# allenai/satlas-super-resolution

Measured on AMD Instinct MI355X. Metric: G+D train-step images/sec, higher is better.
Workload: dtype fp32h

## Files before the change

satlas_super_resolution_amd/csrc/conv_thin.hip:

```cpp
#include "common.h"
#include <cstdlib>

namespace {

constexpr int CT_TH = 8, CT_TW = 32, CT_PH = CT_TH + 2, CT_PW = CT_TW + 2, CT_NPIX = CT_PH * CT_PW;
typedef __bf16 bf16x2t __attribute__((ext_vector_type(2)));

__device__ __forceinline__ float ct_dot8(const u32x4& a, const u32x4& b, float acc) {
    const unsigned a0 = a.x, a1 = a.y, a2 = a.z, a3 = a.w, b0 = b.x, b1 = b.y, b2 = b.z, b3 = b.w;
    acc = __builtin_amdgcn_fdot2_f32_bf16(__builtin_bit_cast(bf16x2t, a0), __builtin_bit_cast(bf16x2t, b0), acc, false);
    acc = __builtin_amdgcn_fdot2_f32_bf16(__builtin_bit_cast(bf16x2t, a1), __builtin_bit_cast(bf16x2t, b1), acc, false);
    acc = __builtin_amdgcn_fdot2_f32_bf16(__builtin_bit_cast(bf16x2t, a2), __builtin_bit_cast(bf16x2t, b2), acc, false);
    acc = __builtin_amdgcn_fdot2_f32_bf16(__builtin_bit_cast(bf16x2t, a3), __builtin_bit_cast(bf16x2t, b3), acc, false);
    return acc;
}

template <int NCO>
__global__ __launch_bounds__(256) void conv_thin_kernel(const ssr_conv_desc d) {
    extern __shared__ __attribute__((aligned(16))) char smem[];
    const int tid = threadIdx.x;
    const int cin = d.Cin, nvec = cin >> 3;
    const int rowb = cin * 2 + 16;
    const int tiles_x = (d.Gw + CT_TW - 1) / CT_TW, tiles_y = (d.Gh + CT_TH - 1) / CT_TH;
    int b = blockIdx.x;
    const int tx_i = b % tiles_x; b /= tiles_x;
    const int ty_i = b % tiles_y;
    const int n = b / tiles_y;
    const int gy0 = ty_i * CT_TH, gx0 = tx_i * CT_TW;
    const __bf16* __restrict__ xg = reinterpret_cast<const __bf16*>(d.x.p);
    const __bf16* __restrict__ wg = reinterpret_cast<const __bf16*>(d.w);
    {
        constexpr int NSV = (CT_NPIX * 8 + 255) / 256;
        const int total = CT_NPIX * nvec;
        const float rn = 1.0f / (float)nvec;
        u32x4 sv[NSV];
        unsigned okm = 0;
#pragma unroll
        for (int q = 0; q < NSV; ++q) {
            const int v = tid + q * 256;
            const int pix = (int)(((float)v + 0.5f) * rn), part = v - pix * nvec;
            const int py = pix / CT_PW, px = pix - py * CT_PW;
            const int ly = gy0 + py - 1, lx = gx0 + px - 1;
            const bool ok = v < total && ly >= 0 && ly < d.Hi && lx >= 0 && lx < d.Wi;
            okm |= ok ? 1u << q : 0u;
            sv[q] = *reinterpret_cast<const u32x4*>(xg + (ok ? ((size_t)(n * d.Hi + ly) * d.Wi + lx) * d.x.cs + d.x.coff + part * 8 : (size_t)0));
        }
#pragma unroll
        for (int q = 0; q < NSV; ++q) {
            const int v = tid + q * 256;
            const int pix = (int)(((float)v + 0.5f) * rn), part = v - pix * nvec;
            if (v < total) *reinterpret_cast<u32x4*>(smem + pix * rowb + part * 16) = (okm >> q) & 1u ? sv[q] : u32x4{0u, 0u, 0u, 0u};
        }
    }
    __syncthreads();
    const int ty = tid >> 5, tx = tid & 31;
    float acc[NCO];
#pragma unroll
    for (int c = 0; c < NCO; ++c) acc[c] = 0.f;
    const char* pb = smem + (ty * CT_PW + tx) * rowb;
    for (int tap = 0; tap < 9; ++tap) {
        const char* pr = pb + ((tap / 3) * CT_PW + tap % 3) * rowb;
        for (int k = 0; k < nvec; ++k) {
            const u32x4 xv = *reinterpret_cast<const u32x4*>(pr + k * 16);
            const __bf16* wk = wg + ((size_t)((k >> 2) * 9 + tap) * d.CoutPad) * 32 + (k & 3) * 8;
#pragma unroll
            for (int c = 0; c < NCO; ++c) {
                const u32x4 wv = *reinterpret_cast<const u32x4*>(wk + c * 32);
                acc[c] = ct_dot8(xv, wv, acc[c]);
            }
        }
    }
    const int gy = gy0 + ty, gx = gx0 + tx;
    if (gy >= d.Gh || gx >= d.Gw) return;
    const size_t pp = (size_t)(n * d.Ho + gy * d.oys + d.oyo) * d.Wo + gx * d.oxs + d.oxo;
    __bf16* __restrict__ yp = reinterpret_cast<__bf16*>(d.y.p);
    __bf16* __restrict__ y0p = reinterpret_cast<__bf16*>(d.y0.p);
    __bf16* __restrict__ y1p = reinterpret_cast<__bf16*>(d.y1.p);
    const __bf16* __restrict__ r1p = reinterpret_cast<const __bf16*>(d.r1.p);
    const __bf16* __restrict__ r2p = reinterpret_cast<const __bf16*>(d.r2.p);
    const __bf16* __restrict__ mp = reinterpret_cast<const __bf16*>(d.m.p);
#pragma unroll
    for (int c = 0; c < NCO; ++c) {
        if (c >= d.Cout) break;
        float v = acc[c] + (d.bias ? d.bias[c] : 0.f);
        if (d.act == SSR_ACT_LRELU) v = lrelu(v);
        v *= d.alpha;
        if (y0p) y0p[pp * d.y0.cs + d.y0.coff + c] = (__bf16)v;
        if (r1p && c < d.r1_nc) v += d.beta1 * (float)r1p[pp * d.r1.cs + d.r1.coff + c];
        if (r2p && c < d.r2_nc) v += d.beta2 * (float)r2p[pp * d.r2.cs + d.r2.coff + c];
        if (d.accumulate) v += (float)yp[pp * d.y.cs + d.y.coff + c];
        if (y1p) y1p[pp * d.y1.cs + d.y1.coff + c] = (__bf16)v;
        if (mp && c >= d.m_c0 && c < d.m_c1) v *= lrelu_grad_from_out((float)mp[pp * d.m.cs + d.m.coff + c]);
        yp[pp * d.y.cs + d.y.coff + c] = (__bf16)v;
    }
}

constexpr int CTF_CB = 32, CTF_ROWB = CTF_CB * 4 + 16;
constexpr int CTF_PATCH = CT_NPIX * CTF_ROWB;

template <int NCO, int X3>
__global__ __launch_bounds__(256) void conv_thin_f32_kernel(const ssr_conv_desc d) {
    constexpr int NCOP = NCO == 1 ? 1 : NCO <= 4 ? 4 : 8;
    extern __shared__ __attribute__((aligned(16))) char smem[];
    float* wl = reinterpret_cast<float*>(smem + CTF_PATCH);
    const int tid = threadIdx.x;
    const int cin = d.Cin, cin16 = (cin + 15) & ~15;
    const int tiles_x = (d.Gw + CT_TW - 1) / CT_TW, tiles_y = (d.Gh + CT_TH - 1) / CT_TH;
    int b = blockIdx.x;
    const int tx_i = b % tiles_x; b /= tiles_x;
    const int ty_i = b % tiles_y;
    const int n = b / tiles_y;
    const int gy0 = ty_i * CT_TH, gx0 = tx_i * CT_TW;
    const float* __restrict__ xg = reinterpret_cast<const float*>(d.x.p);
    const char* __restrict__ wg = reinterpret_cast<const char*>(d.w);
    const int ty = tid >> 5, tx = tid & 31;
    const char* pb = smem + (ty * CT_PW + tx) * CTF_ROWB;
    float acc[NCOP];
#pragma unroll
    for (int c = 0; c < NCOP; ++c) acc[c] = 0.f;
    constexpr int NSV = (CT_NPIX * 8 + 255) / 256;
    int sofs[NSV];
#pragma unroll
    for (int q = 0; q < NSV; ++q) {
        const int v = tid + q * 256, pix = v >> 3;
        const int py = pix / CT_PW, px = pix - py * CT_PW;
        const int ly = gy0 + py - 1, lx = gx0 + px - 1;
        const bool ok = v < CT_NPIX * 8 && ly >= 0 && ly < d.Hi && lx >= 0 && lx < d.Wi;
        sofs[q] = ok ? ((n * d.Hi + ly) * d.Wi + lx) * d.x.cs + d.x.coff + (v & 7) * 4 : -1;
    }
    u32x4 sv[NSV];
    auto load_pass = [&](int c0) {
#pragma unroll
        for (int q = 0; q < NSV; ++q) {
            const bool ok = sofs[q] >= 0 && c0 + ((tid + q * 256) & 7) * 4 < cin;
            sv[q] = *reinterpret_cast<const u32x4*>(xg + (ok ? sofs[q] + c0 : 0));
        }
    };
    auto store_pass = [&](int c0) {
#pragma unroll
        for (int q = 0; q < NSV; ++q) {
            const int v = tid + q * 256;
            const bool ok = sofs[q] >= 0 && c0 + (v & 7) * 4 < cin;
            if (v < CT_NPIX * 8) *reinterpret_cast<u32x4*>(smem + (v >> 3) * CTF_ROWB + (v & 7) * 16) = ok ? sv[q] : u32x4{0u, 0u, 0u, 0u};
        }
    };
    load_pass(0);
    for (int e = tid; e < 9 * cin16 * NCOP; e += 256) {
        const int c = e % NCOP, q = e / NCOP, ci = q % cin16, tap = q / cin16;
        float w = 0.f;
        if (c < NCO) {
            const char* row = wg + ((size_t)((ci >> 4) * 9 + tap) * d.CoutPad + c) * 64;
            if (X3 == 2) {
                const _Float16 h = reinterpret_cast<const _Float16*>(row)[ci & 15], l = reinterpret_cast<const _Float16*>(row)[16 + (ci & 15)];
                w = ((float)h + (float)l) * SSR_F32H_UNSCALE;
            } else if (X3 == 1) {
                const unsigned short h = reinterpret_cast<const unsigned short*>(row)[ci & 15], l = reinterpret_cast<const unsigned short*>(row)[16 + (ci & 15)];
                w = __builtin_bit_cast(float, (unsigned)h << 16) + __builtin_bit_cast(float, (unsigned)l << 16);
            } else {
                w = reinterpret_cast<const float*>(row)[ci & 15];
            }
        }
        wl[e] = w;
    }
    store_pass(0);
    __syncthreads();
    for (int c0 = 0; c0 < cin; c0 += CTF_CB) {
        const bool more = c0 + CTF_CB < cin;
        if (more) load_pass(c0 + CTF_CB);
        const int nk = (min(cin16 - c0, CTF_CB)) >> 2;
        for (int tap = 0; tap < 9; ++tap) {
            const char* pr = pb + ((tap / 3) * CT_PW + tap % 3) * CTF_ROWB;
            const float* wt = wl + (tap * cin16 + c0) * NCOP;
            for (int k = 0; k < nk; ++k) {
                const f32x4 xv = *reinterpret_cast<const f32x4*>(pr + k * 16);
                if constexpr (NCOP == 1) {
                    const f32x4 w = *reinterpret_cast<const f32x4*>(wt + 4 * k);
                    acc[0] = fmaf(xv.x, w.x, acc[0]); acc[0] = fmaf(xv.y, w.y, acc[0]);
                    acc[0] = fmaf(xv.z, w.z, acc[0]); acc[0] = fmaf(xv.w, w.w, acc[0]);
                } else {
#pragma unroll
                    for (int j = 0; j < 4; ++j) {
                        const float xj = j == 0 ? xv.x : j == 1 ? xv.y : j == 2 ? xv.z : xv.w;
#pragma unroll
                        for (int c4 = 0; c4 < NCOP / 4; ++c4) {
                            const f32x4 w = *reinterpret_cast<const f32x4*>(wt + (4 * k + j) * NCOP + 4 * c4);
                            acc[4 * c4] = fmaf(xj, w.x, acc[4 * c4]); acc[4 * c4 + 1] = fmaf(xj, w.y, acc[4 * c4 + 1]);
                            acc[4 * c4 + 2] = fmaf(xj, w.z, acc[4 * c4 + 2]); acc[4 * c4 + 3] = fmaf(xj, w.w, acc[4 * c4 + 3]);
                        }
                    }
                }
            }
        }
        if (more) {
            __syncthreads();
            store_pass(c0 + CTF_CB);
            __syncthreads();
        }
    }
    const int gy = gy0 + ty, gx = gx0 + tx;
    if (gy >= d.Gh || gx >= d.Gw) return;
    const size_t pp = (size_t)(n * d.Ho + gy * d.oys + d.oyo) * d.Wo + gx * d.oxs + d.oxo;
    float* __restrict__ yp = reinterpret_cast<float*>(d.y.p);
    float* __restrict__ y0p = reinterpret_cast<float*>(d.y0.p);
    float* __restrict__ y1p = reinterpret_cast<float*>(d.y1.p);
    const float* __restrict__ r1p = reinterpret_cast<const float*>(d.r1.p);
    const float* __restrict__ r2p = reinterpret_cast<const float*>(d.r2.p);
    const float* __restrict__ mp = reinterpret_cast<const float*>(d.m.p);
#pragma unroll
    for (int c = 0; c < NCO; ++c) {
        if (c >= d.Cout) break;
        float v = acc[c] + (d.bias ? d.bias[c] : 0.f);
        if (d.act == SSR_ACT_LRELU) v = lrelu(v);
        else if (d.act == SSR_ACT_RELU) v = fmaxf(v, 0.f);
        v *= d.alpha;
        if (y0p) y0p[pp * d.y0.cs + d.y0.coff + c] = v;
        if (r1p && c < d.r1_nc) v += d.beta1 * r1p[pp * d.r1.cs + d.r1.coff + c];
        if (r2p && c < d.r2_nc) v += d.beta2 * r2p[pp * d.r2.cs + d.r2.coff + c];
        if (d.accumulate) v += yp[pp * d.y.cs + d.y.coff + c];
        if (y1p) y1p[pp * d.y1.cs + d.y1.coff + c] = v;
        if (mp && c >= d.m_c0 && c < d.m_c1) {
            const float mv = mp[pp * d.m.cs + d.m.coff + c];
            v *= d.m_relu ? (mv > 0.f ? 1.f : 0.f) : lrelu_grad_from_out(mv);
        }
        yp[pp * d.y.cs + d.y.coff + c] = v;
    }
}

template <int NCO, int X3>
int launch_thin_f32(const ssr_conv_desc& d, hipStream_t st) {
    constexpr int NCOP = NCO == 1 ? 1 : NCO <= 4 ? 4 : 8;
    const size_t lds = (size_t)CTF_PATCH + (size_t)9 * ((d.Cin + 15) & ~15) * NCOP * 4;
    auto kern = conv_thin_f32_kernel<NCO, X3>;
    static bool attr_done[SSR_MAX_DEVICES] = {};
    const int attr_dev = ssr_device_ordinal();
    if (!attr_done[attr_dev]) {
        hipError_t e = hipFuncSetAttribute(reinterpret_cast<const void*>(kern), hipFuncAttributeMaxDynamicSharedMemorySize, CTF_PATCH + 9 * 64 * 8 * 4);
        if (e != hipSuccess) return (int)e;
        attr_done[attr_dev] = true;
    }
    const int tiles = d.N * ((d.Gh + CT_TH - 1) / CT_TH) * ((d.Gw + CT_TW - 1) / CT_TW);
    hipLaunchKernelGGL(kern, dim3(tiles), dim3(256), lds, st, d);
    SSR_LAUNCH_CHECK();
    return SSR_OK;
}
template <int X3>
int launch_thin_f32_by_cout(const ssr_conv_desc& d, hipStream_t st) {
    if (d.Cout == 1) return launch_thin_f32<1, X3>(d, st);
    if (d.Cout <= 3) return launch_thin_f32<3, X3>(d, st);
    if (d.Cout == 4) return launch_thin_f32<4, X3>(d, st);
    return launch_thin_f32<8, X3>(d, st);
}

template <int NCO>
int launch_thin(const ssr_conv_desc& d, hipStream_t st) {
    const size_t lds = (size_t)CT_NPIX * (d.Cin * 2 + 16);
// ... 50 lines not shown
```

satlas_super_resolution_amd/csrc/misc.hip:

```cpp
#include "common.h"
#include "adam.h"
#include <cstdlib>

namespace {

__device__ __forceinline__ float wave_sum(float v) {
#pragma unroll
    for (int o = 32; o > 0; o >>= 1) v += __shfl_down(v, o, 64);
    return v;
}
__device__ __forceinline__ float block_sum(float v, float* sh) {
    const int lane = threadIdx.x & 63, w = threadIdx.x >> 6, nw = (blockDim.x + 63) >> 6;
    v = wave_sum(v);
    __syncthreads();
    if (lane == 0) sh[w] = v;
    __syncthreads();
    float s = 0.f;
    if (threadIdx.x < 64) {
        s = (threadIdx.x < nw) ? sh[threadIdx.x] : 0.f;
        s = wave_sum(s);
        if (threadIdx.x == 0) sh[0] = s;
    }
    __syncthreads();
    return sh[0];
}

template <typename T, int X3>
__device__ __forceinline__ void put_packed(T* __restrict__ dst, size_t idx, int ck, float v) {
    if (X3 == 2 && ck == 16) {
        _Float16* row = reinterpret_cast<_Float16*>(dst) + (idx >> 4) * 32;
        const float vs = v * SSR_F32H_WSCALE;
        const _Float16 h = (_Float16)vs;
        row[idx & 15] = h;
        row[16 + (idx & 15)] = (_Float16)(vs - (float)h);
    } else if (X3 == 1 && ck == 16) {
        __bf16* row = reinterpret_cast<__bf16*>(dst) + (idx >> 4) * 32;
        const __bf16 h = (__bf16)v;
        row[idx & 15] = h;
        row[16 + (idx & 15)] = (__bf16)(v - (float)h);
    } else {
        dst[idx] = from_f32<T>(v);
    }
}

template <typename T, int X3 = 0>
__global__ __launch_bounds__(256) void pack_kernel(const ssr_pack_item* __restrict__ items) {
    const ssr_pack_item it = items[blockIdx.y];
    const int KK = it.KH * it.KW;
    const float inv = it.inv_scale ? 1.0f / it.inv_scale[0] : 1.0f;
    const int stride = gridDim.x * blockDim.x;
    const int t0 = blockIdx.x * blockDim.x + threadIdx.x;
    if (it.dst_fwd) {
        T* __restrict__ dst = reinterpret_cast<T*>(it.dst_fwd);
        const int ck = it.ck_fwd, total = it.CoutPad * it.CinPad;
        for (int t = t0; t < total; t += stride) {
            const int cc = t % ck, q = t / ck;
            const int co = q % it.CoutPad, chunk = q / it.CoutPad;
            const int ci = chunk * ck + cc;
            const bool ok = co < it.Cout && ci < it.Cin;
            const float* __restrict__ sp = it.src + ((size_t)co * it.Cin + ci) * KK;
            if (it.fwd_s2d) {
                const int nch = it.CinPad / ck;
                for (int tap = 0; tap < 16; ++tap) {
                    const int ky = tap >> 2, kx = tap & 3, q = (ky & 1) * 2 + (kx & 1), tt = (ky >> 1) * 2 + (kx >> 1);
                    put_packed<T, X3>(dst, ((((size_t)q * nch + chunk) * 4 + tt) * it.CoutPad + co) * ck + cc, ck, ok ? sp[tap] * inv : 0.f);
                }
                continue;
            }
            const size_t dp = ((size_t)chunk * KK * it.CoutPad + co) * ck + cc;
            for (int tap = 0; tap < KK; ++tap) put_packed<T, X3>(dst, dp + (size_t)tap * it.CoutPad * ck, ck, ok ? sp[tap] * inv : 0.f);
        }
    }
    if (it.dst_dgrad) {
        T* __restrict__ dst = reinterpret_cast<T*>(it.dst_dgrad);
        const int ck = it.ck_dgrad, total = it.CinPadO * it.CoutPadI;
        for (int t = t0; t < total; t += stride) {
            const int cc = t % ck, q = t / ck;
            const int o = q % it.CinPadO, chunk = q / it.CinPadO;
            const int k = chunk * ck + cc;
            const bool ok = k < it.Cout && o < it.Cin;
            const float* __restrict__ sp = it.src + ((size_t)k * it.Cin + o) * KK;
            if (it.stride == 1) {
                const size_t dp = ((size_t)chunk * KK * it.CinPadO + o) * ck + cc;
                for (int tap = 0; tap < KK; ++tap)
                    put_packed<T, X3>(dst, dp + (size_t)tap * it.CinPadO * ck, ck, ok ? sp[KK - 1 - tap] * inv : 0.f);
            } else {
                const size_t per_cls = (size_t)4 * it.CinPadO * it.CoutPadI;
                for (int cls = 0; cls < 4; ++cls)
                    for (int tt = 0; tt < 4; ++tt) {
                        const int py = cls >> 1, px = cls & 1, ty = tt >> 1, tx = tt & 1;
                        const int ky = py ? 2 - 2 * ty : 3 - 2 * ty, kx = px ? 2 - 2 * tx : 3 - 2 * tx;
                        put_packed<T, X3>(dst, cls * per_cls + (((size_t)chunk * 4 + tt) * it.CinPadO + o) * ck + cc, ck,
                                          ok ? sp[ky * 4 + kx] * inv : 0.f);
                    }
            }
        }
    }
}

template <typename T, int X3 = 0>
__global__ __launch_bounds__(256) void pack_seg_kernel(const ssr_pack_seg* __restrict__ items) {
    const ssr_pack_seg it = items[blockIdx.y];
    T* __restrict__ dst = reinterpret_cast<T*>(it.dst);
    const int total = it.Cout * it.rows_pad;
    for (int t = blockIdx.x * blockDim.x + threadIdx.x; t < total; t += gridDim.x * blockDim.x) {
        const int kk = t % it.Cout, o = t / it.Cout;
        const int k = it.kbase + kk, chunk = k / it.ck, cc = k - chunk * it.ck;
        const bool ok = o < it.nci;
        const float* __restrict__ sp = it.src + ((size_t)kk * it.Cin + it.ci0 + o) * 9;
        const size_t dp = ((size_t)chunk * 9 * it.rows_pad + o) * it.ck + cc;
#pragma unroll
        for (int tap = 0; tap < 9; ++tap) put_packed<T, X3>(dst, dp + (size_t)tap * it.rows_pad * it.ck, it.ck, ok ? it.scale * sp[8 - tap] : 0.f);
    }
}

template <typename T>
__global__ __launch_bounds__(256) void add_views_kernel(ssr_view dst, ssr_view src, long npix, int C) {
    T* __restrict__ d = reinterpret_cast<T*>(dst.p);
    const T* __restrict__ s = reinterpret_cast<const T*>(src.p);
    const long total = npix * C;
    for (long e = (long)blockIdx.x * blockDim.x + threadIdx.x; e < total; e += (long)gridDim.x * blockDim.x) {
        const long p = e / C;
        const int c = (int)(e - p * C);
        const long di = p * dst.cs + dst.coff + c;
        d[di] = from_f32<T>(to_f32(d[di]) + to_f32(s[p * src.cs + src.coff + c]));
    }
}

template <typename T>
__global__ __launch_bounds__(256) void nchw_to_nhwc_kernel(const float* __restrict__ src, int N, int C, int H, int W,
                                                           ssr_view dst, int s, int up, float scale) {
    const int C2 = C * s * s, H2 = H / s * up, W2 = W / s * up;
    const long total = (long)N * H2 * W2 * C2;
    T* __restrict__ d = reinterpret_cast<T*>(dst.p);
    for (long e = (long)blockIdx.x * blockDim.x + threadIdx.x; e < total; e += (long)gridDim.x * blockDim.x) {
        const int c2 = (int)(e % C2);
        long q = e / C2;
        const int x = (int)(q % W2); q /= W2;
        const int y = (int)(q % H2);
        const int n = (int)(q / H2);
        const int ys = y / up, xs = x / up;
        const int c = c2 / (s * s), i = (c2 / s) % s, j = c2 % s;
        const float v = src[(((long)n * C + c) * H + ys * s + i) * W + xs * s + j] * scale;
        d[(((long)n * H2 + y) * W2 + x) * dst.cs + dst.coff + c2] = from_f32<T>(v);
    }
}

template <typename T>
__global__ __launch_bounds__(256) void nhwc_to_nchw_kernel(ssr_view src, float* __restrict__ dst, int N, int C, int H,
                                                           int W) {
    const long total = (long)N * C * H * W;
    const T* __restrict__ s = reinterpret_cast<const T*>(src.p);
    for (long e = (long)blockIdx.x * blockDim.x + threadIdx.x; e < total; e += (long)gridDim.x * blockDim.x) {
        const int x = (int)(e % W);
        long q = e / W;
        const int y = (int)(q % H); q /= H;
        const int c = (int)(q % C);
        const int n = (int)(q / C);
        dst[e] = to_f32(s[(((long)n * H + y) * W + x) * src.cs + src.coff + c]);
    }
}

template <typename T>
__global__ __launch_bounds__(256) void fill_kernel(T* __restrict__ p, long n, float v) {
    for (long e = (long)blockIdx.x * blockDim.x + threadIdx.x; e < n; e += (long)gridDim.x * blockDim.x)
        p[e] = from_f32<T>(v);
}

__device__ __forceinline__ void bil_src(int o, int n_in, int& i0, int& i1, float& l0, float& l1) {
    float s = 0.5f * (float)o - 0.25f;
    s = s < 0.f ? 0.f : s;
    i0 = (int)s;
    i1 = i0 + (i0 < n_in - 1 ? 1 : 0);
    l1 = s - (float)i0;
    l0 = 1.f - l1;
}

template <typename T> struct VecIO;
template <> struct VecIO<float> {
    static constexpr int N = 4;
    static __device__ __forceinline__ void load(const float* p, float (&f)[4]) {
        const f32x4 v = *reinterpret_cast<const f32x4*>(p);
#pragma unroll
        for (int k = 0; k < 4; ++k) f[k] = v[k];
    }
    static __device__ __forceinline__ void store(float* p, const float (&f)[4]) {
        f32x4 v;
#pragma unroll
        for (int k = 0; k < 4; ++k) v[k] = f[k];
        *reinterpret_cast<f32x4*>(p) = v;
    }
};
template <> struct VecIO<__bf16> {
    static constexpr int N = 8;
    static __device__ __forceinline__ void load(const __bf16* p, float (&f)[8]) {
        const bf16x8 v = *reinterpret_cast<const bf16x8*>(p);
// ... 371 lines not shown
            const float cu = coef * it.u[i];
            const f32x4 g = s4[e], v = v4[j];
            f32x4 o = d4[e];
            o.x += g.x * inv - cu * v.x; o.y += g.y * inv - cu * v.y; o.z += g.z * inv - cu * v.z; o.w += g.w * inv - cu * v.w;
            d4[e] = o;
        }
    } else {
        for (long e = (long)blockIdx.x * blockDim.x + threadIdx.x; e < n; e += (long)gridDim.x * blockDim.x) {
            const int i = (int)(e / it.cols), j = (int)(e - (long)i * it.cols);
            it.dw[e] += it.dw_sn[e] * inv - coef * it.u[i] * it.v[j];
        }
    }
}

template <typename T>
__global__ __launch_bounds__(256) void l1_loss_kernel(ssr_view a, ssr_view b, ssr_view grad, long npix, int C,
                                                      float weight, float* __restrict__ loss_out, bool det) {
    __shared__ float sh[16];
    const long total = npix * C;
    const float invn = 1.f / (float)total;
    const T* __restrict__ ap = reinterpret_cast<const T*>(a.p);
    const T* __restrict__ bp = reinterpret_cast<const T*>(b.p);
    T* __restrict__ gp = reinterpret_cast<T*>(grad.p);
    float s = 0.f;
    for (long e = (long)blockIdx.x * blockDim.x + threadIdx.x; e < total; e += (long)gridDim.x * blockDim.x) {
        const long p = e / C;
        const int c = (int)(e - p * C);
        const float d = to_f32(ap[p * a.cs + a.coff + c]) - to_f32(bp[p * b.cs + b.coff + c]);
        s += fabsf(d);
        if (gp) gp[p * grad.cs + grad.coff + c] = from_f32<T>(d > 0.f ? weight * invn : (d < 0.f ? -weight * invn : 0.f));
    }
    s = block_sum(s, sh);
    if (threadIdx.x == 0 && loss_out) { if (det) loss_out[blockIdx.x] += s * weight * invn; else atomicAdd(loss_out, s * weight * invn); }
}

template <typename T>
__global__ __launch_bounds__(256) void bce_loss_kernel(ssr_view x, ssr_view grad, long npix, float target,
                                                       float weight, float* __restrict__ loss_out,
                                                       float* __restrict__ mean_out, bool det) {
    __shared__ float sh[16];
    const float invn = 1.f / (float)npix;
    const T* __restrict__ xp = reinterpret_cast<const T*>(x.p);
    T* __restrict__ gp = reinterpret_cast<T*>(grad.p);
    float s = 0.f, sm = 0.f;
    for (long p = (long)blockIdx.x * blockDim.x + threadIdx.x; p < npix; p += (long)gridDim.x * blockDim.x) {
        const float v = to_f32(xp[p * x.cs + x.coff]);
        s += fmaxf(v, 0.f) - v * target + log1pf(expf(-fabsf(v)));
        sm += v;
        if (gp) {
            const float sig = 1.f / (1.f + expf(-v));
            gp[p * grad.cs + grad.coff] = from_f32<T>((sig - target) * weight * invn);
        }
    }
    s = block_sum(s, sh);
    if (threadIdx.x == 0 && loss_out) { if (det) loss_out[blockIdx.x] += s * weight * invn; else atomicAdd(loss_out, s * weight * invn); }
    if (mean_out) {
        sm = block_sum(sm, sh);
        if (threadIdx.x == 0) { if (det) mean_out[blockIdx.x] += sm * invn; else atomicAdd(mean_out, sm * invn); }
    }
}

__global__ __launch_bounds__(256) void adam_kernel(const ssr_adam_args a) { adam_update(a); }
__global__ void bump_kernel(int32_t* step) { step[0] += 1; }

__global__ __launch_bounds__(256) void axpby_kernel(float a, const float* __restrict__ x, float b,
                                                    float* __restrict__ y, long n) {
    for (long e = (long)blockIdx.x * blockDim.x + threadIdx.x; e < n; e += (long)gridDim.x * blockDim.x)
        y[e] = a * x[e] + (b == 0.f ? 0.f : b * y[e]);
}

inline int grid_for(long total, int per_block = 256, int cap = 4096) {
    long g = (total + per_block - 1) / per_block;
    if (g < 1) g = 1;
    if (g > cap) g = cap;
    return (int)g;
}

}

#define ST(s) reinterpret_cast<hipStream_t>(s)

extern "C" int ssr_pack_weights(const ssr_pack_item* items_dev, int32_t n_items, int32_t dtype, void* stream) {
    if (!items_dev || n_items <= 0) return SSR_EINVAL;
    dim3 grid(n_items <= 16 ? 1024 : 64, n_items);
    if (dtype == SSR_F32) hipLaunchKernelGGL(pack_kernel<float>, grid, dim3(256), 0, ST(stream), items_dev);
    else if (dtype == SSR_F32X3) hipLaunchKernelGGL((pack_kernel<float, 1>), grid, dim3(256), 0, ST(stream), items_dev);
    else if (dtype == SSR_F32H) hipLaunchKernelGGL((pack_kernel<float, 2>), grid, dim3(256), 0, ST(stream), items_dev);
    else if (dtype == SSR_BF16) hipLaunchKernelGGL(pack_kernel<__bf16>, grid, dim3(256), 0, ST(stream), items_dev);
    else return SSR_EUNSUP;
    SSR_LAUNCH_CHECK();
    return SSR_OK;
}

extern "C" int ssr_pack_dgrad_gather(const ssr_pack_seg* items_dev, int32_t n_items, int32_t dtype, void* stream) {
    if (!items_dev || n_items <= 0) return SSR_EINVAL;
    dim3 grid(8, n_items);
    if (dtype == SSR_F32) hipLaunchKernelGGL(pack_seg_kernel<float>, grid, dim3(256), 0, ST(stream), items_dev);
    else if (dtype == SSR_F32X3) hipLaunchKernelGGL((pack_seg_kernel<float, 1>), grid, dim3(256), 0, ST(stream), items_dev);
    else if (dtype == SSR_BF16) hipLaunchKernelGGL(pack_seg_kernel<__bf16>, grid, dim3(256), 0, ST(stream), items_dev);
    else return SSR_EUNSUP;
    SSR_LAUNCH_CHECK();
    return SSR_OK;
}

extern "C" int ssr_add_views(ssr_view dst, ssr_view src, int32_t dtype, int64_t npix, int32_t C, void* stream) {
    if (dtype == SSR_F32X3) dtype = SSR_F32;
    if (!dst.p || !src.p || npix <= 0 || C <= 0) return SSR_EINVAL;
    const int g = grid_for(npix * C, 256 * 4, 2048);
    if (dtype == SSR_F32)
        hipLaunchKernelGGL(add_views_kernel<float>, dim3(g), dim3(256), 0, ST(stream), dst, src, (long)npix, C);
    else if (dtype == SSR_BF16)
        hipLaunchKernelGGL(add_views_kernel<__bf16>, dim3(g), dim3(256), 0, ST(stream), dst, src, (long)npix, C);
    else return SSR_EUNSUP;
    SSR_LAUNCH_CHECK();
    return SSR_OK;
}

extern "C" int ssr_nchw_to_nhwc(const float* src, int32_t N, int32_t C, int32_t H, int32_t W, ssr_view dst,
                                int32_t dtype, int32_t unshuffle, int32_t up, float scale, void* stream) {
    if (dtype == SSR_F32X3) dtype = SSR_F32;
    if (!src || !dst.p || unshuffle < 1 || up < 1 || H % unshuffle || W % unshuffle) return SSR_EINVAL;
    const long total = (long)N * C * H * W * up * up;
    if (dtype == SSR_F32)
        hipLaunchKernelGGL(nchw_to_nhwc_kernel<float>, dim3(grid_for(total)), dim3(256), 0, ST(stream), src, N, C, H, W,
                           dst, unshuffle, up, scale);
    else if (dtype == SSR_BF16)
        hipLaunchKernelGGL(nchw_to_nhwc_kernel<__bf16>, dim3(grid_for(total)), dim3(256), 0, ST(stream), src, N, C, H,
                           W, dst, unshuffle, up, scale);
    else return SSR_EUNSUP;
    SSR_LAUNCH_CHECK();
    return SSR_OK;
}

extern "C" int ssr_nhwc_to_nchw(ssr_view src, int32_t dtype, float* dst, int32_t N, int32_t C, int32_t H, int32_t W,
                                void* stream) {
    if (dtype == SSR_F32X3) dtype = SSR_F32;
    if (!src.p || !dst) return SSR_EINVAL;
    const long total = (long)N * C * H * W;
    if (dtype == SSR_F32)
        hipLaunchKernelGGL(nhwc_to_nchw_kernel<float>, dim3(grid_for(total)), dim3(256), 0, ST(stream), src, dst, N, C,
                           H, W);
    else if (dtype == SSR_BF16)
        hipLaunchKernelGGL(nhwc_to_nchw_kernel<__bf16>, dim3(grid_for(total)), dim3(256), 0, ST(stream), src, dst, N, C,
                           H, W);
    else return SSR_EUNSUP;
    SSR_LAUNCH_CHECK();
    return SSR_OK;
}

extern "C" int ssr_fill(void* p, int64_t n, int32_t dtype, float value, void* stream) {
    if (dtype == SSR_F32X3) dtype = SSR_F32;
    if (!p || n < 0) return SSR_EINVAL;
    if (n == 0) return SSR_OK;
    if (dtype == SSR_F32)
        hipLaunchKernelGGL(fill_kernel<float>, dim3(grid_for(n)), dim3(256), 0, ST(stream), (float*)p, (long)n, value);
    else if (dtype == SSR_BF16)
        hipLaunchKernelGGL(fill_kernel<__bf16>, dim3(grid_for(n)), dim3(256), 0, ST(stream), (__bf16*)p, (long)n, value);
    else return SSR_EUNSUP;
    SSR_LAUNCH_CHECK();
    return SSR_OK;
}

static const bool g_bilinear_flat_env = [] { const char* e = getenv("SSR_BILINEAR_FLAT"); return e && e[0] == '1'; }();

extern "C" int ssr_bilinear2x_fwd(ssr_view a, ssr_view b, ssr_view y, int32_t dtype, int32_t N, int32_t H, int32_t W,
                                  int32_t C, void* stream) {
    const bool g_bilinear_flat = g_bilinear_flat_env || (dtype & SSR_BILINEAR_FLAT) != 0;
    dtype &= ~SSR_BILINEAR_FLAT;
    if (dtype == SSR_F32X3) dtype = SSR_F32;
    if (!a.p || !y.p || (C % 8) != 0 || (a.cs % 8) || (a.coff % 8) || (y.cs % 8) || (y.coff % 8) ||
        (b.p && ((b.cs % 8) || (b.coff % 8))))
        return SSR_EINVAL;
    const long total = (long)N * H * W * C / (dtype == SSR_F32 ? 4 : 8);
    if (total >= (1L << 31)) return SSR_EINVAL;
    const dim3 tgrid(N * ((H + BF_IH - 1) / BF_IH) * ((W + BF_IW - 1) / BF_IW), dtype == SSR_F32 ? C / 32 : C / 64);
    if (dtype == SSR_F32 && (C % 32) == 0 && !g_bilinear_flat)
        hipLaunchKernelGGL(bilinear2x_fwd_tile_kernel<float>, tgrid, dim3(256), 0, ST(stream), a, b, y, N, H, W);
    else if (dtype == SSR_F32)
        hipLaunchKernelGGL(bilinear2x_fwd_kernel<float>, dim3(grid_for(total, 256, 8192)), dim3(256), 0, ST(stream), a,
                           b, y, N, H, W, C);
    else if (dtype == SSR_BF16 && (C % 64) == 0 && !g_bilinear_flat)
        hipLaunchKernelGGL(bilinear2x_fwd_tile_kernel<__bf16>, tgrid, dim3(256), 0, ST(stream), a, b, y, N, H, W);
// ... 276 lines not shown
```

Measured before the change: 1182.

## Vectorize weight packing and thin-conv weight staging; skip zero high output lanes

The weight pack kernels now process eight input channels per thread, using vector loads and packed 16-byte stores instead of scalar per-element scatter, and launch with 64-thread blocks. The thin conv kernel stages weights into shared memory with coalesced vector loads from the packed layout, replacing the per-element gather. When NCOP is 8, a block-wide OR checks whether the upper four output channels are all zero and, if so, runs a 4-wide inner loop. The aim is to cut per-step weight repacking and staging overhead, at the cost of more code paths, higher register use and alignment-dependent fallbacks.

```diff
diff --git a/satlas_super_resolution_amd/csrc/conv_thin.hip b/satlas_super_resolution_amd/csrc/conv_thin.hip
--- a/satlas_super_resolution_amd/csrc/conv_thin.hip
+++ b/satlas_super_resolution_amd/csrc/conv_thin.hip
@@ -5,6 +5,7 @@
 
 constexpr int CT_TH = 8, CT_TW = 32, CT_PH = CT_TH + 2, CT_PW = CT_TW + 2, CT_NPIX = CT_PH * CT_PW;
 typedef __bf16 bf16x2t __attribute__((ext_vector_type(2)));
+typedef uint32_t u32x2 __attribute__((ext_vector_type(2)));
 
 __device__ __forceinline__ float ct_dot8(const u32x4& a, const u32x4& b, float acc) {
     const unsigned a0 = a.x, a1 = a.y, a2 = a.z, a3 = a.w, b0 = b.x, b1 = b.y, b2 = b.z, b3 = b.w;
@@ -145,25 +146,55 @@
         }
     };
     load_pass(0);
-    for (int e = tid; e < 9 * cin16 * NCOP; e += 256) {
-        const int c = e % NCOP, q = e / NCOP, ci = q % cin16, tap = q / cin16;
-        float w = 0.f;
-        if (c < NCO) {
-            const char* row = wg + ((size_t)((ci >> 4) * 9 + tap) * d.CoutPad + c) * 64;
-            if (X3 == 2) {
-                const _Float16 h = reinterpret_cast<const _Float16*>(row)[ci & 15], l = reinterpret_cast<const _Float16*>(row)[16 + (ci & 15)];
-                w = ((float)h + (float)l) * SSR_F32H_UNSCALE;
-            } else if (X3 == 1) {
-                const unsigned short h = reinterpret_cast<const unsigned short*>(row)[ci & 15], l = reinterpret_cast<const unsigned short*>(row)[16 + (ci & 15)];
-                w = __builtin_bit_cast(float, (unsigned)h << 16) + __builtin_bit_cast(float, (unsigned)l << 16);
+    int hi_nz = 0;
+    {
+        constexpr int NQ = (4 * 9 * NCO * 4 + 255) / 256;
+        const int nq = (cin16 >> 4) * 9 * NCO * 4;
+        unsigned ra[NQ], rb[NQ], rc[NQ], rd[NQ];
+#pragma unroll
+        for (int i = 0; i < NQ; ++i) {
+            const int u = tid + i * 256, r = u >> 2, ct = r / NCO, c = r - ct * NCO;
+            const char* row = wg + (u < nq ? ((size_t)ct * d.CoutPad + c) * 64 : (size_t)0);
+            if (X3 == 0) {
+                const u32x4 t = *reinterpret_cast<const u32x4*>(row + (u & 3) * 16);
+                ra[i] = t.x; rb[i] = t.y; rc[i] = t.z; rd[i] = t.w;
             } else {
-                w = reinterpret_cast<const float*>(row)[ci & 15];
-            }
-        }
-        wl[e] = w;
+                const u32x2 h = *reinterpret_cast<const u32x2*>(row + (u & 3) * 8), l = *reinterpret_cast<const u32x2*>(row + 32 + (u & 3) * 8);
+                ra[i] = h.x; rb[i] = h.y; rc[i] = l.x; rd[i] = l.y;
+            }
+        }
+        if (NCO < NCOP)
+            for (int e = tid; e < 9 * cin16; e += 256)
+#pragma unroll
+                for (int c = NCO; c < NCOP; ++c) wl[e * NCOP + c] = 0.f;
+#pragma unroll
+        for (int i = 0; i < NQ; ++i) {
+            const int u = tid + i * 256, r = u >> 2, ct = r / NCO, c = r - ct * NCO, chunk = ct / 9, tap = ct - chunk * 9;
+            float w[4];
+            if (X3 == 0) {
+                w[0] = __builtin_bit_cast(float, ra[i]); w[1] = __builtin_bit_cast(float, rb[i]);
+                w[2] = __builtin_bit_cast(float, rc[i]); w[3] = __builtin_bit_cast(float, rd[i]);
+            } else {
+#pragma unroll
+                for (int j = 0; j < 4; ++j) {
+                    const unsigned hw = j < 2 ? ra[i] : rb[i], lw = j < 2 ? rc[i] : rd[i];
+                    const unsigned short h = (unsigned short)(j & 1 ? hw >> 16 : hw & 0xffffu), l = (unsigned short)(j & 1 ? lw >> 16 : lw & 0xffffu);
+                    if (X3 == 2) w[j] = ((float)__builtin_bit_cast(_Float16, h) + (float)__builtin_bit_cast(_Float16, l)) * SSR_F32H_UNSCALE;
+                    else w[j] = __builtin_bit_cast(float, (unsigned)h << 16) + __builtin_bit_cast(float, (unsigned)l << 16);
+                }
+            }
+            if (u < nq) {
+                float* wq = wl + (tap * cin16 + chunk * 16 + (u & 3) * 4) * NCOP + c;
+#pragma unroll
+                for (int j = 0; j < 4; ++j) wq[j * NCOP] = w[j];
+                if (NCOP == 8 && c >= 4 && (w[0] != 0.f || w[1] != 0.f || w[2] != 0.f || w[3] != 0.f)) hi_nz = 1;
+            }
+        }
     }
     store_pass(0);
-    __syncthreads();
+    bool wide = true;
+    if constexpr (NCOP == 8) wide = __syncthreads_or(hi_nz) != 0;
+    else __syncthreads();
     for (int c0 = 0; c0 < cin; c0 += CTF_CB) {
         const bool more = c0 + CTF_CB < cin;
         if (more) load_pass(c0 + CTF_CB);
@@ -171,6 +202,19 @@
         for (int tap = 0; tap < 9; ++tap) {
             const char* pr = pb + ((tap / 3) * CT_PW + tap % 3) * CTF_ROWB;
             const float* wt = wl + (tap * cin16 + c0) * NCOP;
+            if (NCOP == 8 && !wide) {
+                for (int k = 0; k < nk; ++k) {
+                    const f32x4 xv = *reinterpret_cast<const f32x4*>(pr + k * 16);
+#pragma unroll
+                    for (int j = 0; j < 4; ++j) {
+                        const float xj = j == 0 ? xv.x : j == 1 ? xv.y : j == 2 ? xv.z : xv.w;
+                        const f32x4 w = *reinterpret_cast<const f32x4*>(wt + (4 * k + j) * NCOP);
+                        acc[0] = fmaf(xj, w.x, acc[0]); acc[1] = fmaf(xj, w.y, acc[1]);
+                        acc[2] = fmaf(xj, w.z, acc[2]); acc[3] = fmaf(xj, w.w, acc[3]);
+                    }
+                }
+                continue;
+            }
             for (int k = 0; k < nk; ++k) {
                 const f32x4 xv = *reinterpret_cast<const f32x4*>(pr + k * 16);
                 if constexpr (NCOP == 1) {
diff --git a/satlas_super_resolution_amd/csrc/misc.hip b/satlas_super_resolution_amd/csrc/misc.hip
--- a/satlas_super_resolution_amd/csrc/misc.hip
+++ b/satlas_super_resolution_amd/csrc/misc.hip
@@ -43,14 +43,10 @@
     }
 }
 
-template <typename T, int X3 = 0>
-__global__ __launch_bounds__(256) void pack_kernel(const ssr_pack_item* __restrict__ items) {
-    const ssr_pack_item it = items[blockIdx.y];
+template <typename T, int X3>
+__device__ void pack_item_elems(const ssr_pack_item& it, float inv, int t0, int stride, bool fwd, bool dgrad) {
     const int KK = it.KH * it.KW;
-    const float inv = it.inv_scale ? 1.0f / it.inv_scale[0] : 1.0f;
-    const int stride = gridDim.x * blockDim.x;
-    const int t0 = blockIdx.x * blockDim.x + threadIdx.x;
-    if (it.dst_fwd) {
+    if (fwd) {
         T* __restrict__ dst = reinterpret_cast<T*>(it.dst_fwd);
         const int ck = it.ck_fwd, total = it.CoutPad * it.CinPad;
         for (int t = t0; t < total; t += stride) {
@@ -71,7 +67,7 @@
             for (int tap = 0; tap < KK; ++tap) put_packed<T, X3>(dst, dp + (size_t)tap * it.CoutPad * ck, ck, ok ? sp[tap] * inv : 0.f);
         }
     }
-    if (it.dst_dgrad) {
+    if (dgrad) {
         T* __restrict__ dst = reinterpret_cast<T*>(it.dst_dgrad);
         const int ck = it.ck_dgrad, total = it.CinPadO * it.CoutPadI;
         for (int t = t0; t < total; t += stride) {
@@ -98,9 +94,8 @@
     }
 }
 
-template <typename T, int X3 = 0>
-__global__ __launch_bounds__(256) void pack_seg_kernel(const ssr_pack_seg* __restrict__ items) {
-    const ssr_pack_seg it = items[blockIdx.y];
+template <typename T, int X3>
+__device__ void pack_seg_elems(const ssr_pack_seg& it) {
     T* __restrict__ dst = reinterpret_cast<T*>(it.dst);
     const int total = it.Cout * it.rows_pad;
     for (int t = blockIdx.x * blockDim.x + threadIdx.x; t < total; t += gridDim.x * blockDim.x) {
@@ -112,6 +107,170 @@
 #pragma unroll
         for (int tap = 0; tap < 9; ++tap) put_packed<T, X3>(dst, dp + (size_t)tap * it.rows_pad * it.ck, it.ck, ok ? it.scale * sp[8 - tap] : 0.f);
     }
+}
+
+__device__ __forceinline__ bool al16(const void* p) { return (reinterpret_cast<uintptr_t>(p) & 15) == 0; }
+__device__ __forceinline__ unsigned pk16(unsigned short a, unsigned short b) { return (unsigned)a | ((unsigned)b << 16); }
+
+template <int KK>
+__device__ __forceinline__ void load_oct(const float* __restrict__ sp, size_t rstride, int nval, float mul, float (&v)[8 * KK]) {
+    if (nval == 8 && rstride == (size_t)KK && al16(sp)) {
+#pragma unroll
+        for (int i = 0; i < 2 * KK; ++i) {
+            const f32x4 x = reinterpret_cast<const f32x4*>(sp)[i];
+            v[4 * i] = x.x * mul; v[4 * i + 1] = x.y * mul; v[4 * i + 2] = x.z * mul; v[4 * i + 3] = x.w * mul;
+        }
+        return;
+    }
+#pragma unroll
+    for (int e = 0; e < 8; ++e) {
+        const float* __restrict__ r = sp + e * rstride;
+        if (e >= nval) {
+#pragma unroll
+            for (int t = 0; t < KK; ++t) v[e * KK + t] = 0.f;
+        } else if (KK % 4 == 0 && al16(r)) {
+#pragma unroll
+            for (int i = 0; i < KK / 4; ++i) {
+                const f32x4 x = reinterpret_cast<const f32x4*>(r)[i];
+                v[e * KK + 4 * i] = x.x * mul; v[e * KK + 4 * i + 1] = x.y * mul; v[e * KK + 4 * i + 2] = x.z * mul; v[e * KK + 4 * i + 3] = x.w * mul;
+            }
+        } else {
+#pragma unroll
+            for (int t = 0; t < KK; ++t) v[e * KK + t] = r[t] * mul;
+        }
+    }
+}
+
+template <typename T, int X3>
+__device__ __forceinline__ void put_oct(T* __restrict__ dst, size_t row, int ck, int o8, const float (&w)[8]) {
+    if (X3 != 0 && ck == 16) {
+        unsigned short h[8], l[8];
+#pragma unroll
+        for (int e = 0; e < 8; ++e) {
+            if (X3 == 2) {
+                const float vs = w[e] * SSR_F32H_WSCALE;
+                const _Float16 hh = (_Float16)vs;
+                h[e] = __builtin_bit_cast(unsigned short, hh);
+                l[e] = __builtin_bit_cast(unsigned short, (_Float16)(vs - (float)hh));
+            } else {
+                const __bf16 hh = (__bf16)w[e];
+                h[e] = __builtin_bit_cast(unsigned short, hh);
+                l[e] = __builtin_bit_cast(unsigned short, (__bf16)(w[e] - (float)hh));
+            }
+        }
+        char* r = reinterpret_cast<char*>(dst) + row * 64 + o8 * 16;
+        *reinterpret_cast<u32x4*>(r) = u32x4{pk16(h[0], h[1]), pk16(h[2], h[3]), pk16(h[4], h[5]), pk16(h[6], h[7])};
+        *reinterpret_cast<u32x4*>(r + 32) = u32x4{pk16(l[0], l[1]), pk16(l[2], l[3]), pk16(l[4], l[5]), pk16(l[6], l[7])};
+    } else if (sizeof(T) == 4) {
+        float* r = reinterpret_cast<float*>(dst) + row * ck + o8 * 8;
+        *reinterpret_cast<f32x4*>(r) = f32x4{w[0], w[1], w[2], w[3]};
+        *reinterpret_cast<f32x4*>(r + 4) = f32x4{w[4], w[5], w[6], w[7]};
+    } else {
+        unsigned short b[8];
+#pragma unroll
+        for (int e = 0; e < 8; ++e) b[e] = __builtin_bit_cast(unsigned short, (__bf16)w[e]);
+        *reinterpret_cast<u32x4*>(reinterpret_cast<char*>(dst) + (row * ck + o8 * 8) * 2) =
+            u32x4{pk16(b[0], b[1]), pk16(b[2], b[3]), pk16(b[4], b[5]), pk16(b[6], b[7])};
+    }
+}
+
+template <typename T, int X3, int KK>
+__device__ void pack_item_rows(const ssr_pack_item& it, float inv, int t0, int stride, bool fwd, bool dgrad) {
+    float v[8 * KK], w[8];
+    if (fwd) {
+        T* __restrict__ dst = reinterpret_cast<T*>(it.dst_fwd);
+        const int ck = it.ck_fwd, opr = ck >> 3, nch = it.CinPad / ck, total = it.CoutPad * (it.CinPad >> 3);
+        for (int u = t0; u < total; u += stride) {
+            const int o8 = u % opr, q = u / opr;
+            const int co = q % it.CoutPad, chunk = q / it.CoutPad;
+            const int ci0 = chunk * ck + o8 * 8;
+            const int nval = co < it.Cout ? max(0, min(8, it.Cin - ci0)) : 0;
+            load_oct<KK>(it.src + ((size_t)co * it.Cin + ci0) * KK, (size_t)KK, nval, inv, v);
+#pragma unroll
+            for (int tap = 0; tap < KK; ++tap) {
+#pragma unroll
+                for (int e = 0; e < 8; ++e) w[e] = v[e * KK + tap];
+                size_t row = ((size_t)chunk * KK + tap) * it.CoutPad + co;
+                if (KK == 16 && it.fwd_s2d) {
+                    const int ky = tap >> 2, kx = tap & 3, pq = (ky & 1) * 2 + (kx & 1), tt = (ky >> 1) * 2 + (kx >> 1);
+                    row = (((size_t)pq * nch + chunk) * 4 + tt) * it.CoutPad + co;
+                }
+                put_oct<T, X3>(dst, row, ck, o8, w);
+            }
+        }
+    }
+    if (dgrad) {
+        T* __restrict__ dst = reinterpret_cast<T*>(it.dst_dgrad);
+        const int ck = it.ck_dgrad, opr = ck >> 3, total = it.CinPadO * (it.CoutPadI >> 3);
+        const size_t cls_rows = (size_t)4 * it.CinPadO * (it.CoutPadI / ck);
+        for (int u = t0; u < total; u += stride) {
+            const int o = u % it.CinPadO, ko = u / it.CinPadO;
+            const int chunk = ko / opr, o8 = ko - chunk * opr, k0 = ko * 8;
+            const int nval = o < it.Cin ? max(0, min(8, it.Cout - k0)) : 0;
+            load_oct<KK>(it.src + ((size_t)k0 * it.Cin + o) * KK, (size_t)it.Cin * KK, nval, inv, v);
+            if (it.stride == 1) {
+#pragma unroll
+                for (int tap = 0; tap < KK; ++tap) {
+#pragma unroll
+                    for (int e = 0; e < 8; ++e) w[e] = v[e * KK + KK - 1 - tap];
+                    put_oct<T, X3>(dst, ((size_t)chunk * KK + tap) * it.CinPadO + o, ck, o8, w);
+                }
+            } else if (KK == 16) {
+#pragma unroll
+                for (int cls = 0; cls < 4; ++cls)
+#pragma unroll
+                    for (int tt = 0; tt < 4; ++tt) {
+                        const int py = cls >> 1, px = cls & 1, ty = tt >> 1, tx = tt & 1;
+                        const int ky = py ? 2 - 2 * ty : 3 - 2 * ty, kx = px ? 2 - 2 * tx : 3 - 2 * tx;
+#pragma unroll
+                        for (int e = 0; e < 8; ++e) w[e] = v[e * KK + (ky * 4 + kx) % KK];
+                        put_oct<T, X3>(dst, cls * cls_rows + ((size_t)chunk * 4 + tt) * it.CinPadO + o, ck, o8, w);
+                    }
+            }
+        }
+    }
+}
+
+template <typename T, int X3 = 0>
+__global__ __launch_bounds__(256) void pack_kernel(const ssr_pack_item* __restrict__ items) {
+    const ssr_pack_item it = items[blockIdx.y];
+    const int KK = it.KH * it.KW;
+    const float inv = it.inv_scale ? 1.0f / it.inv_scale[0] : 1.0f;
+    const int stride = gridDim.x * blockDim.x;
+    const int t0 = blockIdx.x * blockDim.x + threadIdx.x;
+    const bool fwd = it.dst_fwd != nullptr, dgrad = it.dst_dgrad != nullptr;
+    const bool rows_f = fwd && (KK == 9 || KK == 16) && (it.ck_fwd & 7) == 0 && (it.CinPad % it.ck_fwd) == 0 && al16(it.dst_fwd) &&
+                        (!it.fwd_s2d || KK == 16);
+    const bool rows_d = dgrad && (KK == 9 || KK == 16) && (it.ck_dgrad & 7) == 0 && (it.CoutPadI % it.ck_dgrad) == 0 && al16(it.dst_dgrad) &&
+                        (it.stride == 1 || KK == 16);
+    if (KK == 9) pack_item_rows<T, X3, 9>(it, inv, t0, stride, rows_f, rows_d);
+    else if (KK == 16) pack_item_rows<T, X3, 16>(it, inv, t0, stride, rows_f, rows_d);
+    pack_item_elems<T, X3>(it, inv, t0, stride, fwd && !rows_f, dgrad && !rows_d);
+}
+
+template <typename T, int X3>
+__device__ void pack_seg_rows(const ssr_pack_seg& it) {
+    T* __restrict__ dst = reinterpret_cast<T*>(it.dst);
+    float v[72], w[8];
+    const int total = it.rows_pad * (it.Cout >> 3);
+    for (int u = blockIdx.x * blockDim.x + threadIdx.x; u < total; u += gridDim.x * blockDim.x) {
+        const int o = u % it.rows_pad, j = u / it.rows_pad;
+        const int k0 = it.kbase + 8 * j, chunk = k0 / it.ck, o8 = (k0 - chunk * it.ck) >> 3;
+        load_oct<9>(it.src + ((size_t)(8 * j) * it.Cin + it.ci0 + o) * 9, (size_t)it.Cin * 9, o < it.nci ? 8 : 0, it.scale, v);
+#pragma unroll
+        for (int tap = 0; tap < 9; ++tap) {
+#pragma unroll
+            for (int e = 0; e < 8; ++e) w[e] = v[e * 9 + 8 - tap];
+            put_oct<T, X3>(dst, ((size_t)chunk * 9 + tap) * it.rows_pad + o, it.ck, o8, w);
+        }
+    }
+}
+
+template <typename T, int X3 = 0>
+__global__ __launch_bounds__(256) void pack_seg_kernel(const ssr_pack_seg* __restrict__ items) {
+    const ssr_pack_seg it = items[blockIdx.y];
+    if ((it.Cout & 7) == 0 && (it.kbase & 7) == 0 && (it.ck & 7) == 0 && al16(it.dst)) pack_seg_rows<T, X3>(it);
+    else pack_seg_elems<T, X3>(it);
 }
 
 template <typename T>
@@ -649,11 +808,11 @@
 
 extern "C" int ssr_pack_weights(const ssr_pack_item* items_dev, int32_t n_items, int32_t dtype, void* stream) {
     if (!items_dev || n_items <= 0) return SSR_EINVAL;
-    dim3 grid(n_items <= 16 ? 1024 : 64, n_items);
-    if (dtype == SSR_F32) hipLaunchKernelGGL(pack_kernel<float>, grid, dim3(256), 0, ST(stream), items_dev);
-    else if (dtype == SSR_F32X3) hipLaunchKernelGGL((pack_kernel<float, 1>), grid, dim3(256), 0, ST(stream), items_dev);
-    else if (dtype == SSR_F32H) hipLaunchKernelGGL((pack_kernel<float, 2>), grid, dim3(256), 0, ST(stream), items_dev);
-    else if (dtype == SSR_BF16) hipLaunchKernelGGL(pack_kernel<__bf16>, grid, dim3(256), 0, ST(stream), items_dev);
+    dim3 grid(n_items <= 16 ? 512 : 32, n_items);
+    if (dtype == SSR_F32) hipLaunchKernelGGL(pack_kernel<float>, grid, dim3(64), 0, ST(stream), items_dev);
+    else if (dtype == SSR_F32X3) hipLaunchKernelGGL((pack_kernel<float, 1>), grid, dim3(64), 0, ST(stream), items_dev);
+    else if (dtype == SSR_F32H) hipLaunchKernelGGL((pack_kernel<float, 2>), grid, dim3(64), 0, ST(stream), items_dev);
+    else if (dtype == SSR_BF16) hipLaunchKernelGGL(pack_kernel<__bf16>, grid, dim3(64), 0, ST(stream), items_dev);
     else return SSR_EUNSUP;
     SSR_LAUNCH_CHECK();
     return SSR_OK;
@@ -662,9 +821,9 @@
 extern "C" int ssr_pack_dgrad_gather(const ssr_pack_seg* items_dev, int32_t n_items, int32_t dtype, void* stream) {
     if (!items_dev || n_items <= 0) return SSR_EINVAL;
     dim3 grid(8, n_items);
-    if (dtype == SSR_F32) hipLaunchKernelGGL(pack_seg_kernel<float>, grid, dim3(256), 0, ST(stream), items_dev);
-    else if (dtype == SSR_F32X3) hipLaunchKernelGGL((pack_seg_kernel<float, 1>), grid, dim3(256), 0, ST(stream), items_dev);
-    else if (dtype == SSR_BF16) hipLaunchKernelGGL(pack_seg_kernel<__bf16>, grid, dim3(256), 0, ST(stream), items_dev);
+    if (dtype == SSR_F32) hipLaunchKernelGGL(pack_seg_kernel<float>, grid, dim3(64), 0, ST(stream), items_dev);
+    else if (dtype == SSR_F32X3) hipLaunchKernelGGL((pack_seg_kernel<float, 1>), grid, dim3(64), 0, ST(stream), items_dev);
+    else if (dtype == SSR_BF16) hipLaunchKernelGGL(pack_seg_kernel<__bf16>, grid, dim3(64), 0, ST(stream), items_dev);
     else return SSR_EUNSUP;
     SSR_LAUNCH_CHECK();
     return SSR_OK;
```

After: 1184, median of 6. No clear change (+0.2%).
